# dotchen/LAV

Measured on AMD Instinct MI355X. Metric: frames/s full agent fwd (32k-pt LiDAR + 3 cams), higher is better.
Workload: dtype f32 (convolution contractions on the matrix cores with f32 accumulate at the error of an fp32 dot product, DESIGN 4.3: the layers on the split-operand kernel - BEV backbone, heads, crop stems, the brake net's mid-size layers - and ERFNet's persistent runs of pairs as two power-of-two-scaled fp16 pie

## Files before the change

### include/lav_amd.h

```cpp
#ifndef LAV_AMD_H
#define LAV_AMD_H

#include <stddef.h>
#include <stdint.h>

#ifdef __cplusplus
extern "C" {
#endif

#define LAV_ABI_VERSION 46

#define LAV_OK 0
#define LAV_EINVAL (-1)
#define LAV_EHIP (-2)
#define LAV_EWORKSPACE (-3)

int lav_abi_version(void);
const char *lav_last_error(void);
int lav_device_count(void);

int lav_profile_enable(int slots);
int lav_profile_reset(void);
int lav_profile_read(const char *kernel, double *total_ms, int *launches);

typedef struct lav_grid {
    float min_x, max_x, min_y, max_y;
    float ppm;
    int nx, ny;
} lav_grid;

typedef struct lav_pointnet {
    const float *w1, *b1, *w2, *b2;
    int num_input;
    int channels;
} lav_pointnet;

size_t lav_pillar_workspace_bytes(int batch, int max_points, const lav_grid *grid);
int lav_pillar_workspace_init(void *workspace, size_t workspace_bytes, void *stream);

int lav_pillar_scatter(const float *points, const int *h_num_points, int batch, int max_points, int D,
                       const lav_grid *grid, const lav_pointnet *net, float *canvas,
                       int *unique_coords, int *inverse, int *counts,
                       void *workspace, size_t workspace_bytes, void *stream);
int lav_pillar_amax_count(int batch, const lav_grid *grid);
int lav_pillar_scatter_amax(const float *points, const int *h_num_points, int batch, int max_points, int D,
                            const lav_grid *grid, const lav_pointnet *net, float *canvas,
                            int *unique_coords, int *inverse, int *counts, float *amax_parts,
                            void *workspace, size_t workspace_bytes, void *stream);

typedef struct lav_camera {
    float K[9];
    float l2w[16];
    float w2c[16];
} lav_camera;

int lav_paint(const float *lidar, int n, int lidar_dim, const float *sem, int ncam, int sem_c, int h, int w,
              const lav_camera *h_cams, float *fused, int *uvz, void *stream);

int lav_gru_cast(const float *embd, int B, int embd_dim, int H, int num_cmds, int T,
                 const float *w_ih, const float *w_hh, const float *b_ih, const float *b_hh,
                 const float *mlp_w, const float *mlp_b, float *out,
                 void *workspace, size_t workspace_bytes, void *stream);
size_t lav_gru_cast_workspace_bytes(int B, int embd_dim, int H, int num_cmds, int T);
// ... 141 lines not shown
int lav_bn_train_amax_count(int batch, int channels, long plane);
int lav_bn_train_forward_amax(const float *x, const float *residual, float *y, int batch, int channels, long plane, const float *gamma,
                              const float *beta, double eps, int relu_pre, int relu_post, float *save_mean, float *save_var,
                              float *save_rstd, float *amax_y, void *workspace, size_t workspace_bytes, void *stream);
int lav_bn_train_backward_amax(const float *x, const float *y, const float *dy, int batch, int channels, long plane, const float *gamma,
                               const float *save_mean, const float *save_rstd, int relu_pre, int relu_post, float *dx, float *dres,
                               float *dgamma, float *dbeta, float *amax_dx, void *workspace, size_t workspace_bytes, void *stream);

int lav_bn_train_forward_mask(const float *x, const float *residual, const float *chmask, float *y, int batch, int channels, long plane,
                              const float *gamma, const float *beta, double eps, int relu_post, float *save_mean, float *save_var,
                              float *save_rstd, float *amax_y, void *workspace, size_t workspace_bytes, void *stream);
int lav_bn_train_backward_mask(const float *x, const float *y, const float *dy, const float *chmask, int batch, int channels, long plane,
                               const float *gamma, const float *save_mean, const float *save_rstd, int relu_post, float *dx, float *dres,
                               float *dgamma, float *dbeta, float *amax_dx, void *workspace, size_t workspace_bytes, void *stream);

size_t lav_conv_wgrad_workspace_bytes(int batch, int cin, int cout, int h, int w, int ksize, int stride);
int lav_conv_wgrad(const float *x, const float *dy, int batch, int cin, int cout, int h, int w, int ksize, int stride, float *dw,
                   void *workspace, size_t workspace_bytes, void *stream);
int lav_conv_wgrad_amax(const float *x, const float *dy, int batch, int cin, int cout, int h, int w, int ksize, int stride, float *dw,
                        void *workspace, size_t workspace_bytes, const float *amax_x, int n_amax_x, const float *amax_dy, int n_amax_dy,
                        void *stream);

size_t lav_upconv_pointwise_packed_floats(int cin, int cout, int k);
int lav_upconv_pointwise_pack(int cin, int cout, int k, const float *h_weight, float *h_packed);
int lav_upconv_pointwise_parts(int batch, int cin, int cout, int ih, int iw, int k, int pad, int out_pad);
int lav_upconv_pointwise(int batch, int cin, int cout, int ih, int iw, int k, int pad, int out_pad, const float *x, const float *w_packed,
                         const float *scale, const float *shift, int relu_pre, int out_c_total, int out_c_offset, float *y,
                         float *amax_out, void *stream);

size_t lav_conv1d_pair_packed_weight_floats(int channels);
int lav_conv1d_pair_pack_weights(int channels, const float *h_weight, float *h_packed);
size_t lav_conv1d_pair_chain_workspace_bytes(int batch, int h);
size_t lav_conv1d_pair_chain_lds_bytes(int channels, int w, int d_b_max);
int lav_conv1d_pair_chain(int batch, int channels, int h, int w, int npairs, const int *d_a, const int *d_b, const int *residual,
                          const int *relu_post, const float *x, const float *const *wa_packed, const float *const *bias_a,
                          const float *const *wb_packed, const float *const *bias_b, const float *const *scale,
                          const float *const *shift, float *const *out, void *workspace, size_t workspace_bytes, void *stream);
int lav_conv1d_pair_chain_f16(int batch, int channels, int h, int w, int npairs, const int *d_a, const int *d_b, const int *residual,
                              const int *relu_post, const float *x, const float *const *wa_packed, const float *const *bias_a,
                              const float *const *wb_packed, const float *const *bias_b, const float *const *scale,
                              const float *const *shift, float *const *out, void *workspace, size_t workspace_bytes, void *stream);
int lav_conv1d_pair_chain_region(int row_offset, int clean_rows);
int lav_conv1d_pair_chain_status(const void *workspace, int *h_timeouts_launches2, void *stream);
size_t lav_conv1d_pair_lds_bytes(int channels, int w, int d_b);
size_t lav_conv3x3_run_f16_workspace_bytes(int channels, int h, int w, int nlayers);
size_t lav_conv3x3_run_f16_lds_bytes(int channels, int h, int w);
size_t lav_conv3x3_run_f16_weight_bytes(int channels);
int lav_conv3x3_run_f16_amax_count(int channels, int h, int w);
long lav_conv_f16_weights_offset(const lav_conv *c);
int lav_conv3x3_run_f16(int channels, int h, int w, int nlayers, const float *x, const void *const *w_f16, const float *const *scale,
                        const float *const *shift, float *out, const float *amax_in, int amax_in_count, float *amax_out, void *workspace,
                        size_t workspace_bytes, void *stream);
int lav_conv3x3_run_f16_status(const void *workspace, int *h_timeouts_launches2, void *stream);
size_t lav_conv3x3_tile_f16_lds_bytes(int channels, int h, int w, int nlayers);
int lav_conv3x3_tile_f16_amax_count(int channels, int h, int w, int nlayers);
int lav_conv3x3_tile_f16(int channels, int h, int w, int nlayers, const float *x, const void *const *w_f16, const float *const *scale,
                         const float *const *shift, float *out, const float *amax_in, int amax_in_count, float *amax_out, void *stream);
int lav_conv1d_pair(int batch, int channels, int h, int w, int d_a, int d_b, const float *x, const float *wa_packed,
                    const float *bias_a, const float *wb_packed, const float *bias_b, const float *scale, const float *shift,
                    const float *residual, int relu_post, float *y, void *stream);

int lav_pool_affine(const float *x, int batch, int channels, int h, int w, const float *scale, const float *shift, int relu,
                    float *y, int out_c_total, int out_c_offset, void *stream);

int lav_pair_train_supported(int channels, int width);
size_t lav_pair_train_workspace_bytes(int batch, int channels, int h);
int lav_pair_train_forward(const float *x, const float *wa, const float *ba, const float *wb, const float *bb, int batch, int channels,
                           int h, int w, int dil, float *t, float *z, void *stream);
int lav_pair_train_backward(const float *x, const float *t, const float *dz, const float *wa, const float *wb, int batch, int channels,
                            int h, int w, int dil, float *dt, float *dx, float *dwa, float *dba, float *dwb, float *dbb, void *workspace,
                            size_t workspace_bytes, void *stream);

size_t lav_seg_xent_workspace_bytes(void);
int lav_seg_xent_forward(const float *logits, const long long *labels, int batch, int classes, long plane, float *loss, float *dlogits,
                         void *workspace, size_t workspace_bytes, void *stream);

int lav_seg_xent_up_forward(const float *logits, const void *labels, int label_bytes, int batch, int classes, int h, int w, int scale,
                            float *loss, float *dlogits, void *workspace, size_t workspace_bytes, void *stream);

typedef struct lav_camera_f64 {
    double l2w[16];
    double w2c[16];
    double K[9];
} lav_camera_f64;

int lav_paint_frames(const float *lidar, const int *offsets, int frames, int total, int lidar_dim, const float *sem, int ncam,
                     int sem_c, int h, int w, const lav_camera_f64 *h_cams, float *painted, int *uvz, void *stream);

int lav_image_u8_to_f32(const unsigned char *img, int n, int h, int w, int c_src, int reverse, float *out, void *stream);

enum { LAV_AUG_BLUR = 0, LAV_AUG_NOISE = 1, LAV_AUG_DROPOUT = 2, LAV_AUG_MULTIPLY = 3, LAV_AUG_CONTRAST = 4, LAV_AUG_GRAYSCALE = 5,
       LAV_AUG_ELASTIC = 6, LAV_AUG_OPS = 7 };

typedef struct lav_augment_params {
    int order[7];
    int active;
    int per_channel;
    unsigned sample;
    unsigned tag;
    float blur_sigma;
    float blur_w[5];
    float noise_scale;
    float dropout_p;
    float multiply[3];
    float contrast[3];
    float gray_alpha;
    float elastic_alpha;
    float field_w[5];
} lav_augment_params;

int lav_augment_u8(const unsigned char *in, unsigned char *out, int n, int h, int w, const lav_augment_params *params,
                   unsigned long long seed, void *stream);

int lav_bev_stack_u8(const unsigned char *planes, const double *coef, const int *shift, unsigned char *out, int n, int h, int w,
                     int threshold, void *stream);
int lav_bev_stack_tile_paths(const double *coef, const int *shift, int h, int w, int *counts);
// ... 97 lines not shown
```

### lav_amd/_lib.py

```python
from __future__ import annotations

import ctypes as C
import os

HERE = os.path.dirname(os.path.abspath(__file__))
LIB_PATH = os.environ.get("LAV_AMD_LIB") or os.path.join(HERE, "liblav_amd.so")

ABI_VERSION = 46
MAX_CAM = 4
MAX_CAM_F64 = 8


class Grid(C.Structure):
    _fields_ = [("min_x", C.c_float), ("max_x", C.c_float), ("min_y", C.c_float), ("max_y", C.c_float),
                ("ppm", C.c_float), ("nx", C.c_int), ("ny", C.c_int)]


class PointNet(C.Structure):
    _fields_ = [("w1", C.c_void_p), ("b1", C.c_void_p), ("w2", C.c_void_p), ("b2", C.c_void_p),
                ("num_input", C.c_int), ("channels", C.c_int)]


class Camera(C.Structure):
    _fields_ = [("K", C.c_float * 9), ("l2w", C.c_float * 16), ("w2c", C.c_float * 16)]


class CameraF64(C.Structure):
    _fields_ = [("l2w", C.c_double * 16), ("w2c", C.c_double * 16), ("K", C.c_double * 9)]


class Conv(C.Structure):
    _fields_ = [(n, C.c_int) for n in (
        "batch", "in_c_total", "in_c_offset", "cin", "h", "w", "cout", "kh", "kw", "stride", "pad_h", "pad_w",
        "dil_h", "dil_w", "transposed", "out_pad", "out_c_total", "out_c_offset", "relu_pre", "relu_post", "sigmoid", "target_cus")] + [("pad_value", C.c_float), ("precision", C.c_int)]


CONV_F32, CONV_BF16X6, CONV_F16X3 = 1, 2, 3


_P, _I, _Z, _F = C.c_void_p, C.c_int, C.c_size_t, C.c_float
SIGNATURES = {
    "lav_abi_version": (_I, []),
    "lav_last_error": (C.c_char_p, []),
    "lav_device_count": (_I, []),
    "lav_profile_enable": (_I, [_I]),
    "lav_profile_reset": (_I, []),
    "lav_profile_read": (_I, [C.c_char_p, C.POINTER(C.c_double), C.POINTER(_I)]),
    "lav_pillar_workspace_bytes": (_Z, [_I, _I, C.POINTER(Grid)]),
    "lav_pillar_workspace_init": (_I, [_P, _Z, _P]),
    "lav_pillar_decorate_workspace_bytes": (_Z, [_I, _I, C.POINTER(Grid)]),
    "lav_pillar_scatter": (_I, [_P, C.POINTER(_I), _I, _I, _I, C.POINTER(Grid), C.POINTER(PointNet), _P, _P, _P, _P,
                                _P, _Z, _P]),
    "lav_pillar_amax_count": (_I, [_I, C.POINTER(Grid)]),
    "lav_pillar_scatter_amax": (_I, [_P, C.POINTER(_I), _I, _I, _I, C.POINTER(Grid), C.POINTER(PointNet), _P, _P, _P, _P, _P,
                                     _P, _Z, _P]),
    "lav_paint": (_I, [_P, _I, _I, _P, _I, _I, _I, _I, C.POINTER(Camera), _P, _P, _P]),
    "lav_paint_frames": (_I, [_P, _P, _I, _I, _I, _P, _I, _I, _I, _I, C.POINTER(CameraF64), _P, _P, _P]),
    "lav_image_u8_to_f32": (_I, [_P, _I, _I, _I, _I, _I, _P, _P]),
    "lav_gru_cast": (_I, [_P, _I, _I, _I, _I, _I, _P, _P, _P, _P, _P, _P, _P, _P, _Z, _P]),
    "lav_gru_cast_workspace_bytes": (_Z, [_I, _I, _I, _I, _I]),
    "lav_embed_cast": (_I, [_P, _I, _I, _I, _P, _I, _I, _I, _P, _P, _P, _P, _P, _P, _P, _P, _P, _P, _P, _P, _P]),
# ... 33 lines not shown
    "lav_upconv_pointwise_parts": (_I, [_I] * 8),
    "lav_upconv_pointwise": (_I, [_I] * 8 + [_P, _P, _P, _P, _I, _I, _I, _P, _P, _P]),
    "lav_conv1d_pair_chain_workspace_bytes": (_Z, [_I, _I]),
    "lav_conv1d_pair_chain_region": (_I, [_I, _I]),
    "lav_conv1d_pair_chain_lds_bytes": (_Z, [_I, _I, _I]),
    "lav_conv1d_pair_chain": (_I, [_I, _I, _I, _I, _I, C.POINTER(_I), C.POINTER(_I), C.POINTER(_I), C.POINTER(_I), _P] + [C.POINTER(_P)] * 7 + [_P, _Z, _P]),
    "lav_conv1d_pair_chain_f16": (_I, [_I, _I, _I, _I, _I, C.POINTER(_I), C.POINTER(_I), C.POINTER(_I), C.POINTER(_I), _P] + [C.POINTER(_P)] * 7 + [_P, _Z, _P]),
    "lav_conv1d_pair_chain_status": (_I, [_P, C.POINTER(_I), _P]),
    "lav_conv1d_pair_lds_bytes": (_Z, [_I, _I, _I]),
    "lav_conv3x3_run_f16_workspace_bytes": (_Z, [_I, _I, _I, _I]),
    "lav_conv3x3_run_f16_lds_bytes": (_Z, [_I, _I, _I]),
    "lav_conv3x3_run_f16_weight_bytes": (_Z, [_I]),
    "lav_conv3x3_run_f16_amax_count": (_I, [_I, _I, _I]),
    "lav_conv_f16_weights_offset": (C.c_long, [C.POINTER(Conv)]),
    "lav_conv3x3_run_f16": (_I, [_I, _I, _I, _I, _P, C.POINTER(_P), C.POINTER(_P), C.POINTER(_P), _P, _P, _I, _P, _P, _Z, _P]),
    "lav_conv3x3_run_f16_status": (_I, [_P, C.POINTER(_I), _P]),
    "lav_conv3x3_tile_f16_lds_bytes": (_Z, [_I, _I, _I, _I]),
    "lav_conv3x3_tile_f16_amax_count": (_I, [_I, _I, _I, _I]),
    "lav_conv3x3_tile_f16": (_I, [_I, _I, _I, _I, _P, C.POINTER(_P), C.POINTER(_P), C.POINTER(_P), _P, _P, _I, _P, _P]),
    "lav_conv1d_pair": (_I, [_I, _I, _I, _I, _I, _I, _P, _P, _P, _P, _P, _P, _P, _P, _I, _P, _P]),
    "lav_gru_seq_forward": (_I, [_P, _I, _P, _P, _P, _I, _I, _I, _P, _P, _P]),
    "lav_gru_seq_backward_workspace_bytes": (_Z, [_I, _I]),
    "lav_gru_seq_backward": (_I, [_P, _P, _P, _P, _P, _I, _I, _I, _P, _P, _P, _P, _Z, _P]),
    "lav_bn_train_workspace_bytes": (_Z, [_I]),
    "lav_bn_train_forward_mask": (_I, [_P, _P, _P, _P, _I, _I, C.c_long, _P, _P, C.c_double, _I, _P, _P, _P, _P, _P, _Z, _P]),
    "lav_bn_train_backward_mask": (_I, [_P, _P, _P, _P, _I, _I, C.c_long, _P, _P, _P, _I, _P, _P, _P, _P, _P, _P, _Z, _P]),
    "lav_pair_train_supported": (_I, [_I, _I]),
    "lav_pair_train_workspace_bytes": (_Z, [_I, _I, _I]),
    "lav_pair_train_forward": (_I, [_P, _P, _P, _P, _P, _I, _I, _I, _I, _I, _P, _P, _P]),
    "lav_pair_train_backward": (_I, [_P, _P, _P, _P, _P, _I, _I, _I, _I, _I, _P, _P, _P, _P, _P, _P, _P, _Z, _P]),
    "lav_seg_xent_workspace_bytes": (_Z, []),
    "lav_seg_xent_forward": (_I, [_P, _P, _I, _I, C.c_long, _P, _P, _P, _Z, _P]),
    "lav_seg_xent_up_forward": (_I, [_P, _P, _I, _I, _I, _I, _I, _I, _P, _P, _P, _Z, _P]),
    "lav_attn_train_workspace_bytes": (_Z, [_I, _I, _I, _I]),
    "lav_attn_train_forward": (_I, [_P, _I, _I, _I, _I, _P, _P, _P, _P, C.c_float, _P, _P, _P, _P, _P, _P]),
    "lav_attn_train_backward": (_I, [_P, _I, _I, _I, _I, _P, _P, _P, _P, C.c_float, _P, _P, _P, _P, _P, _P, _P, _P, _P, _Z, _P]),
    "lav_bn_train_forward": (_I, [_P, _P, _P, _I, _I, C.c_long, _P, _P, C.c_double, _I, _I, _P, _P, _P, _P, _Z, _P]),
    "lav_bn_train_backward": (_I, [_P, _P, _P, _I, _I, C.c_long, _P, _P, _P, _I, _I, _P, _P, _P, _P, _P, _Z, _P]),
    "lav_bn_train_amax_count": (_I, [_I, _I, C.c_long]),
    "lav_bn_train_forward_amax": (_I, [_P, _P, _P, _I, _I, C.c_long, _P, _P, C.c_double, _I, _I, _P, _P, _P, _P, _P, _Z, _P]),
    "lav_bn_train_backward_amax": (_I, [_P, _P, _P, _I, _I, C.c_long, _P, _P, _P, _I, _I, _P, _P, _P, _P, _P, _P, _Z, _P]),
    "lav_attn_pool": (_I, [_P, _I, _I, _I, _I, _P, _P, _P, _P, _P, _P]),
    "lav_linear_act": (_I, [_P, _I, _I, _P, _P, _I, _I, _P, _P]),
    "lav_maxpool3x3s2": (_I, [_P, _I, _I, _I, _I, _P, _P]),
    "lav_channel_affine": (_I, [_P, _I, _I, C.c_long, _P, _P, _P, _P]),
    "lav_nonfinite_count": (_I, [_I, C.POINTER(_P), C.POINTER(C.c_long), _P, _P]),
    "lav_copy_many": (_I, [_I, C.POINTER(_P), C.POINTER(_P), C.POINTER(_Z), _P]),
    "lav_stage_many": (_I, [_I, C.POINTER(_P), C.POINTER(_P), C.POINTER(_I), C.POINTER(C.c_long), C.POINTER(_I), _P]),
    "lav_det_decode": (_I, [_P, _I, _I, _I] + [C.c_double] * 10 + [_P, _P, _P]),
    "lav_det_decode_report": (_I, [_P, _I, _I, _I] + [C.c_double] * 10 + [_P, _P, _P, _P, _P, _P]),
    "lav_stage_many_block": (_I, [_I, C.POINTER(_P), C.POINTER(_P), C.POINTER(_I), C.POINTER(C.c_long), C.POINTER(_I), _P, _I, _P, _P]),
    "lav_batch_limit": (_I, [_P]),
    "lav_pool_affine": (_I, [_P, _I, _I, _I, _I, _P, _P, _I, _P, _I, _I, _P]),
    "lav_merge_ticks": (_I, [_P, _P, _I, _I, _P, _P]),
    "lav_stack_sweeps": (_I, [_P, _P, _P, _P, _P, _P, _I, _I, _I, _P, _P]),
    "lav_extract_peaks_workspace_bytes": (_Z, [_I, _I, _I]),
    "lav_extract_peaks": (_I, [_P, _I, _I, _I, _I, _I, _I, _P, _I, _P, _I, _P, _P, _Z, _P]),
    "lav_heads_at_peaks_packed_floats": (_Z, [_I, _I]),
    "lav_heads_at_peaks": (_I, [_P, _I, _I, _I, _P, _I, _I, _I, _P, _P, _P, _P, _P, _P, _P, _P, _P]),
    "lav_augment_u8": (_I, [_P, _P, _I, _I, _I, _P, C.c_ulonglong, _P]),
    "lav_bev_stack_u8": (_I, [_P, _P, _P, _P, _I, _I, _I, _I, _P]),
    "lav_bev_stack_tile_paths": (_I, [C.POINTER(C.c_double), C.POINTER(_I), _I, _I, C.POINTER(_I)]),
    "lav_debug_view": (_I, [_P, _I, _I, _P, _I, _I, _P, _I, _I, _P, _I, _P, _I, _P, _I, _P, _P, _P, C.c_double, C.c_double, _I, C.c_double, C.c_double, _I,
                            _I, _I, _P, _P, _P]),
    "lav_log_view": (_I, [_P, _I, _P, _I, _P, _P, _I, _I, _P, _P, _I, _P, _I, _I, _P, _P]),
    "lav_eval_acc_words": (_Z, [_I]),
    "lav_eval_frame": (_I, [_P, _P, _P, _I, _I, _F, _P, _I, _P, _P, _I, _I, _I, _P, _P, _I, _P, _P, _P, _I] + [C.c_double] * 6 + [_I, _P, _P]),
    "lav_eval_seg": (_I, [_P, _P, _I, _I, _I, _I, _I, _P, _P]),
    "lav_eval_scores": (_I, [_P, _P, _I, C.c_double, _I, _P, _P]),
    "lav_eval_plans_words": (_Z, [_I]),
    "lav_eval_plans": (_I, [_P, _P, _P, _P, _P, _P, _I, _I, _I, _P, _P, _P, _I, _P, _P]),
    "lav_eval_distill_words": (_Z, [_I]),
    "lav_eval_distill": (_I, [_P] * 8 + [_I, _I, _I] + [_P] * 5 + [_I, _P, _P]),
    "lav_eval_drive_words": (_Z, [_I]),
    "lav_eval_drive": (_I, [_P, _P, _P, _I, _I, _I, _I, _P, _P, _I, _P, _P, _I, _I] + [C.c_double] * 6 + [_I, _P, _P]),
    "lav_eval_det_words": (_Z, [_I]),
    "lav_eval_det": (_I, [_P, _I, _P, _P, _I, _I, _I, _P, _P, _I, _I] + [C.c_double] * 6 + [_P, _I, _P, _I, _P, _I, _I, _P, _P]),
    "lav_jpeg_scan_capacity": (C.c_longlong, [_I, _I, _I]),
    "lav_jpeg_workspace_bytes": (_Z, [_I, _I, _I, _I]),
    "lav_jpeg_encode": (_I, [_P, _I, _I, _I, _I, _P, _I, _P, C.c_longlong, _P, _P, _Z, _P]),
    "lav_optim_chunk": (_I, []),
    "lav_optim_workspace_bytes": (_Z, [C.c_longlong, C.c_longlong]),
    "lav_optim_grad_stats": (_I, [_P, _I, _I, _P, _I, _I, _P, C.c_double, _P, _Z, _P]),
    "lav_optim_adam_step": (_I, [_P, _I, _I, _P, _I, _I, _P, _P, C.c_double, _P, _Z, _P]),
}

_lib = None


def load() -> C.CDLL:
    global _lib
    if _lib is not None:
        return _lib
    if not os.path.exists(LIB_PATH):
        raise RuntimeError(
            f"{LIB_PATH} not found: build it with `python -m lav_amd.build` (hipcc, gfx950). "
            "lav_amd has no CPU or pure-torch fallback.")
    lib = C.CDLL(LIB_PATH)
    for name, (res, args) in SIGNATURES.items():
        fn = getattr(lib, name)
        fn.restype = res
        fn.argtypes = args
    got = lib.lav_abi_version()
    if got != ABI_VERSION:
        raise RuntimeError(f"liblav_amd ABI {got} != binding ABI {ABI_VERSION}: rebuild (python -m lav_amd.build --force)")
    _lib = lib
# ... 16 lines not shown
```

### lav_amd/build.py

```python
from __future__ import annotations

import os
import subprocess
import sys
import time

HERE = os.path.dirname(os.path.abspath(__file__))
REPO = os.path.dirname(HERE)
CSRC = os.path.join(HERE, "csrc")
LIB = os.path.join(HERE, "liblav_amd.so")
SOURCES = ["misc.hip", "pillar.hip", "paint.hip", "paint_frames.hip", "gru.hip", "gru_seq.hip", "conv.hip", "conv_f16.hip", "conv_pair.hip", "conv_run.hip", "conv_tile.hip", "deconv.hip", "crop.hip", "frame.hip", "heads_peaks.hip", "attn.hip", "bn_train.hip", "conv_wgrad.hip", "upconv.hip", "conv_pair_train.hip", "augment.hip", "bev_stack.hip", "debug_view.hip", "log_view.hip", "eval_metrics.hip", "eval_camera.hip", "eval_plans.hip", "eval_drive.hip", "eval_distill.hip", "eval_det.hip", "jpeg.hip", "optim.hip"]
EXTRA_FLAGS = {"pillar.hip": ["-ffp-contract=off"], "paint.hip": ["-ffp-contract=off"], "paint_frames.hip": ["-ffp-contract=off"], "crop.hip": ["-ffp-contract=off"],
               "frame.hip": ["-ffp-contract=off"], "augment.hip": ["-ffp-contract=off"], "bev_stack.hip": ["-ffp-contract=off"],
               "debug_view.hip": ["-ffp-contract=off", "-fhip-fp32-correctly-rounded-divide-sqrt"],
               "log_view.hip": ["-ffp-contract=off"],
               "eval_metrics.hip": ["-ffp-contract=off"],
               "eval_plans.hip": ["-ffp-contract=off"],
               "eval_drive.hip": ["-ffp-contract=off"],
               "eval_det.hip": ["-ffp-contract=off"],
               "eval_distill.hip": ["-ffp-contract=off"],
               "optim.hip": ["-ffp-contract=off", "-fhip-fp32-correctly-rounded-divide-sqrt"]}
FLAGS = ["--offload-arch=gfx950", "-O3", "-std=c++17", "-fPIC", "-Wall", "-Wno-unused-function", "-fno-slp-vectorize",
         "-I", os.path.join(REPO, "include"), "-I", CSRC]


def _hipcc() -> str:
    for c in (os.environ.get("HIPCC"), "/opt/rocm/bin/hipcc", "hipcc"):
        if c and (os.path.isabs(c) and os.path.exists(c) or not os.path.isabs(c)):
            return c
    raise RuntimeError("hipcc not found")


def needs_build() -> bool:
    if not os.path.exists(LIB):
        return True
    t = os.path.getmtime(LIB)
    deps = [os.path.join(CSRC, f) for f in os.listdir(CSRC)] + [os.path.join(REPO, "include", "lav_amd.h")]
    return any(os.path.getmtime(d) > t for d in deps)


def build(force: bool = False, verbose: bool = True) -> str:
    if not force and not needs_build():
        return LIB
    objs = []
    procs = []
    os.makedirs(os.path.join(HERE, "build"), exist_ok=True)
    t0 = time.time()
    for s in SOURCES:
        o = os.path.join(HERE, "build", s.replace(".hip", ".o"))
        objs.append(o)
        cmd = [_hipcc(), *FLAGS, *EXTRA_FLAGS.get(s, []), "-c", os.path.join(CSRC, s), "-o", o]
        procs.append((s, subprocess.Popen(cmd, stdout=subprocess.PIPE, stderr=subprocess.STDOUT, text=True)))
    for s, p in procs:
        out, _ = p.communicate()
        if p.returncode != 0:
            raise RuntimeError(f"hipcc failed on {s}:\n{out}")
        if verbose and out.strip():
            print(out)
    link = [_hipcc(), "--offload-arch=gfx950", "-shared", "-fPIC", *objs, "-o", LIB]
    r = subprocess.run(link, stdout=subprocess.PIPE, stderr=subprocess.STDOUT, text=True)
    if r.returncode != 0:
        raise RuntimeError("link failed:\n" + r.stdout)
    if verbose:
        print(f"built {LIB} in {time.time() - t0:.1f}s")
# ... 6 lines not shown
```

### lav_amd/erfnet.py

```python
from __future__ import annotations

import os

import torch
import torch.nn as nn
import torch.nn.functional as F

from . import ops
from .engine import Engine
from .ops import Conv1dPair, Conv1dPairChain, ConvLayer, GroupedDeconv, infer_precision

_USE_PAIRS = os.environ.get("LAV_ERFNET_PAIRS", "1") != "0"


def _affine(bn, sl):
    s, t = ops.bn_fold(bn.running_mean, bn.running_var, bn.weight, bn.bias, bn.eps)
    return s[sl].float()[None, :, None, None].contiguous(), t[sl].float()[None, :, None, None].contiguous()


class DownsamplerBlock(nn.Module):
    def __init__(self, cin, cout):
        super().__init__()
        self.conv = nn.Conv2d(cin, cout - cin, 3, stride=2, padding=1, bias=True)
        self.pool = nn.MaxPool2d(2, stride=2)
        self.bn = nn.BatchNorm2d(cout, eps=1e-3)

    def forward(self, x):
        return F.relu(self.bn(torch.cat([self.conv(x), self.pool(x)], 1)))

    def engine(self, device, input_affine=None):
        from . import ops
        nconv = self.conv.out_channels
        cout = self.bn.num_features
        w, b, pad = self.conv.weight.detach(), self.conv.bias.detach(), 0.0
        s_in, t_in = (1.0, 0.0) if input_affine is None else input_affine
        if input_affine is not None:
            if not s_in > 0:
                raise RuntimeError("input_affine needs a positive scale")
            b = (b.double() + t_in * w.double().sum(dim=(1, 2, 3))).float()
            w = (w.double() * s_in).float()
            pad = -t_in / s_in
        sl = slice(0, nconv)
        bn = tuple(t[sl] for t in (self.bn.running_mean, self.bn.running_var, self.bn.weight, self.bn.bias))
        conv = ConvLayer(w, stride=2, padding=(1, 1), bias=b, bn=bn, bn_eps=self.bn.eps, relu_post=True, out_c_total=cout,
                         pad_value=pad, device=device)
        ps, pt = _affine(self.bn, slice(nconv, cout))
        ps, pt = ps.reshape(-1).double(), pt.reshape(-1).double()
        ps, pt = (ps * s_in).float().to(device), (pt + ps * t_in).float().to(device)

        def run(x):
            out = conv(x)
            return ops.pool_affine(x, ps, pt, out, nconv, relu=True)
        return run


class non_bottleneck_1d(nn.Module):
    def __init__(self, ch, dropprob, dilated):
        super().__init__()
        d = dilated
        self.conv3x1_1 = nn.Conv2d(ch, ch, (3, 1), padding=(1, 0))
        self.conv1x3_1 = nn.Conv2d(ch, ch, (1, 3), padding=(0, 1))
        self.bn1 = nn.BatchNorm2d(ch, eps=1e-3)
        self.conv3x1_2 = nn.Conv2d(ch, ch, (3, 1), padding=(d, 0), dilation=(d, 1))
        self.conv1x3_2 = nn.Conv2d(ch, ch, (1, 3), padding=(0, d), dilation=(1, d))
        self.bn2 = nn.BatchNorm2d(ch, eps=1e-3)
        self.dropout = nn.Dropout2d(dropprob)

    def forward(self, x):
        if self.training and x.is_cuda:
            from .train.hipnn import nb1d_train
            return nb1d_train(self, x)
        return self.forward_torch(x)

    def forward_torch(self, x):
        y = F.relu(self.bn1(self.conv1x3_1(F.relu(self.conv3x1_1(x)))))
        y = self.bn2(self.conv1x3_2(F.relu(self.conv3x1_2(y))))
        if self.dropout.p != 0:
            y = self.dropout(y)
        return F.relu(y + x)

    def engine(self, device):
        a = ConvLayer.from_module(self.conv3x1_1, relu_post=True, device=device)
        b = ConvLayer.from_module(self.conv1x3_1, self.bn1, relu_post=True, device=device)
        c = ConvLayer.from_module(self.conv3x1_2, relu_post=True, device=device)
        d = ConvLayer.from_module(self.conv1x3_2, self.bn2, relu_post=True, device=device)
        p1 = Conv1dPair(self.conv3x1_1, self.conv1x3_1, self.bn1, device=device)
        p2 = Conv1dPair(self.conv3x1_2, self.conv1x3_2, self.bn2, device=device)

        def run(x):
            if _USE_PAIRS and p1.supported(x) and p2.supported(x):
                return p2(p1(x), residual=x)
            return d(c(b(a(x))), residual=x)
        run.pairs = (p1, p2)
        return run


def _chain_blocks(stages):
    out, run = [], []

    def flush():
        if not run:
            return
        blocks = list(run)
        run.clear()
        if len(blocks) == 1 or not _USE_PAIRS:
            out.extend(blocks)
# ... 27 lines not shown
    def __init__(self, cin, cout):
        super().__init__()
        self.conv = nn.ConvTranspose2d(cin, cout, 3, stride=2, padding=1, output_padding=1, bias=True)
        self.bn = nn.BatchNorm2d(cout, eps=1e-3)

    def forward(self, x):
        return F.relu(self.bn(self.conv(x)))

    def engine(self, device):
        return ConvLayer.from_module(self.conv, self.bn, relu_post=True, device=device)


class Encoder(nn.Module):
    def __init__(self, num_classes):
        super().__init__()
        self.initial_block = DownsamplerBlock(3, 16)
        blocks = [DownsamplerBlock(16, 64)] + [non_bottleneck_1d(64, 0.03, 1) for _ in range(5)] + [DownsamplerBlock(64, 128)]
        blocks += [non_bottleneck_1d(128, 0.3, d) for _ in range(2) for d in (2, 4, 8, 16)]
        self.layers = nn.ModuleList(blocks)
        self.output_conv = nn.Conv2d(128, num_classes, 1)

    def forward(self, x, predict=False):
        x = self.initial_block(x)
        for layer in self.layers:
            x = layer(x)
        return self.output_conv(x) if predict else x


class Decoder(nn.Module):
    def __init__(self, num_classes):
        super().__init__()
        self.layers = nn.ModuleList([UpsamplerBlock(128, 64), non_bottleneck_1d(64, 0, 1), non_bottleneck_1d(64, 0, 1),
                                     UpsamplerBlock(64, 16), non_bottleneck_1d(16, 0, 1), non_bottleneck_1d(16, 0, 1)])
        self.output_conv = nn.ConvTranspose2d(16, num_classes, 2, stride=2)

    def forward(self, x):
        for layer in self.layers:
            x = layer(x)
        return self.output_conv(x)


class ERFNet(Engine):
    def __init__(self, num_classes):
        super().__init__()
        self.encoder = Encoder(num_classes)
        self.decoder = Decoder(num_classes)

    _mark_stale = Engine._drop

    def _engine(self, device, input_affine=None, softmax=False):
        def build():
            stages = [self.encoder.initial_block.engine(device, input_affine)]
            stages += [m.engine(device) for m in self.encoder.layers]
            stages += [m.engine(device) for m in self.decoder.layers]
            stages = _chain_blocks(stages)
            stages.append(GroupedDeconv([self.decoder.output_conv], softmax=softmax, device=device))
            return stages
        return self._engine_for(device, (input_affine, softmax, infer_precision()), build)

    def chains(self, precision):
        return [s.chain for key, stages in (self.__dict__.get("_eng") or {}).items() if isinstance(key, tuple) and key[2] == precision
                for s in stages if getattr(s, "chain", None) is not None]

    def forward(self, x, input_affine=None, softmax=False):
        if self.training:
            if input_affine is not None:
                x = x * input_affine[0] + input_affine[1]
            y = self.decoder(self.encoder(x))
            return torch.softmax(y, dim=1) if softmax else y
        if not x.is_cuda:
            raise RuntimeError("ERFNet: eval-mode forward needs a tensor in HBM - lav_amd has no CPU path "
                               "(CPU evaluation for tests and baselines: oracle/camera.py)")
        shared = os.environ.get("LAV_CHAIN_SHARED_CLEAN", "1") != "0"
        cap, off, first = ops.pair_chain_capacity(x.device), 0, True
        for stage in self._engine(x.device, input_affine, softmax):
            chain = getattr(stage, "chain", None)
            rows = x.shape[0] * x.shape[2]
            if shared and chain is not None and chain.supported(x) and off + rows <= cap:
                with ops.pair_chain_region(off, cap if first else 0):
                    x = stage(x)
                off, first = off + rows, False
            else:
                if chain is not None:
                    shared = False
                x = stage(x)
        return x
```

### lav_amd/ops.py

```python
from __future__ import annotations

import ctypes as C
import functools
import os as _os
import threading as _threading
from typing import Optional, Sequence

import numpy as np
import torch

from . import _lib
from ._lib import Camera, Conv, Grid, PointNet, check

_workspaces: dict = {}


def _stream() -> int:
    return torch.cuda.current_stream().cuda_stream


def _ptr(t: Optional[torch.Tensor]) -> Optional[int]:
    return None if t is None else t.data_ptr()


# ... 1573 lines not shown
        nb = bsrc.numel() * bsrc.element_size()
        if (stage and not bsrc.is_cuda and bsrc.is_contiguous() and bdst.is_cuda and bdst.is_contiguous() and nb % 4 == 0 and 0 < nb <= 256
                and nb == bdst.numel() * bdst.element_size() and bdst.data_ptr() % 4 == 0):
            blk = (bsrc.data_ptr(), nb, bdst.data_ptr())
        else:
            bdst.copy_(bsrc, non_blocking=True)
    for i in range(0, len(stage), 8):
        part = stage[i:i + 8]
        n = len(part)
        dims, strides = [], []
        for dst, src in part:
            pad = 4 - src.dim()
            dims += [1] * pad + list(src.shape)
            strides += [0] * pad + list(src.stride())
        b = blk if i == 0 else (None, 0, None)
        check(lib.lav_stage_many_block(n, (C.c_void_p * n)(*[s_.data_ptr() for _, s_ in part]), (C.c_void_p * n)(*[d.data_ptr() for d, _ in part]),
                                       (C.c_int * (4 * n))(*dims), (C.c_long * (4 * n))(*strides),
                                       (C.c_int * n)(*[int(s_.dtype == torch.uint8) for _, s_ in part]), b[0], b[1], b[2], _stream()), "lav_stage_many")


def linear_act(x: torch.Tensor, weight: torch.Tensor, bias, sigmoid: bool = False) -> torch.Tensor:
    x = _f32c(x, "x")
    B, K = x.shape
    O = weight.shape[0]
    out = torch.empty((B, O), dtype=torch.float32, device=x.device)
    check(_lib.load().lav_linear_act(_ptr(x), B, K, _ptr(_f32c(weight, "weight")), _ptr(None if bias is None else _f32c(bias, "bias")), O,
                                     int(bool(sigmoid)), _ptr(out), _stream()), "lav_linear_act")
    return out


def attn_pool(x: torch.Tensor, u: torch.Tensor, dots_bias: torch.Tensor, w_v: torch.Tensor, b_v: torch.Tensor, heads: int,
              out: Optional[torch.Tensor] = None) -> torch.Tensor:
    x = _f32c(x, "x")
    B, Cc, H, W = x.shape
    if out is None:
        out = torch.empty((B, Cc), dtype=torch.float32, device=x.device)
    elif tuple(out.shape) != (B, Cc) or out.dtype != torch.float32 or not out.is_cuda or (B > 1 and out.stride(0) != Cc) or out.stride(1) != 1:
        raise RuntimeError("attn_pool: out must be a (B, C) float32 buffer in HBM with rows C apart")
    check(_lib.load().lav_attn_pool(_ptr(x), B, Cc, H * W, int(heads), _ptr(_f32c(u, "u")), _ptr(_f32c(dots_bias, "dots_bias")),
                                    _ptr(_f32c(w_v, "w_v")), _ptr(_f32c(b_v, "b_v")), _ptr(out), _stream()), "lav_attn_pool")
    return out


def pool_affine(x: torch.Tensor, scale: torch.Tensor, shift: torch.Tensor, out: torch.Tensor, out_c_offset: int, relu: bool = True):
    x = _f32c(x, "x")
    B, Cc, H, W = x.shape
    if out.shape[0] != B or out.shape[2:] != (H // 2, W // 2) or not out.is_contiguous():
        raise RuntimeError("pool_affine: output buffer does not match")
    check(_lib.load().lav_pool_affine(_ptr(x), B, Cc, H, W, _ptr(_f32c(scale, "scale")), _ptr(_f32c(shift, "shift")), int(relu),
                                      _ptr(out), out.shape[1], int(out_c_offset), _stream()), "lav_pool_affine")
    return out


def crop_rotate(features: torch.Tensor, locs: torch.Tensor, oris: torch.Tensor, pixels_per_meter: float, crop: int,
                offset_x: float, offset_y: float) -> torch.Tensor:
    lib = _lib.load()
    features, locs, oris, out = _crop_args(features, locs, oris, crop)
    fb, Cc, H, W = features.shape
    n = locs.shape[0]
    if fb not in (1, n):
        raise RuntimeError("features batch must be 1 (shared map) or N")
    check(lib.lav_crop_rotate(_ptr(features), fb, Cc, H, W, _ptr(locs), _ptr(oris), n, float(pixels_per_meter), int(crop),
                              float(offset_x), float(offset_y), _ptr(out), _stream()), "lav_crop_rotate")
    return out


def merge_ticks(tick: torch.Tensor, prev: torch.Tensor, out: torch.Tensor | None = None) -> torch.Tensor:
    lib = _lib.load()
    tick, prev = _f32c(tick, "tick"), _f32c(prev, "prev")
    if tick.shape != prev.shape or tick.dim() != 2 or tick.shape[1] != 4:
        raise RuntimeError(f"merge_ticks: tick {tuple(tick.shape)} / prev {tuple(prev.shape)} must both be (P, 4)")
    P = tick.shape[0]
    if out is None:
        out = torch.empty((2 * P, 4), dtype=torch.float32, device=tick.device)
    check(lib.lav_merge_ticks(_ptr(tick), _ptr(prev), P, 4, _ptr(out), _stream()), "lav_merge_ticks")
    return out


def stack_sweeps(fused: torch.Tensor, ring: torch.Tensor, slot: torch.Tensor, sweeps: torch.Tensor, R: torch.Tensor,
                 t: torch.Tensor, out: torch.Tensor | None = None) -> torch.Tensor:
    lib = _lib.load()
    fused, ring, R, t = _f32c(fused, "fused"), _f32c(ring, "ring"), _f32c(R, "R"), _f32c(t.reshape(-1, 3), "t")
    S, rows, dim = sweeps.numel(), fused.shape[0], fused.shape[1]
    if ring.shape[1:] != fused.shape or slot.dtype != torch.long or sweeps.dtype != torch.long or R.shape != (S, 3, 3):
        raise RuntimeError("stack_sweeps: inconsistent arguments")
    if out is None:
        out = torch.empty((S * rows, dim + S), dtype=torch.float32, device=fused.device)
    check(lib.lav_stack_sweeps(_ptr(fused), _ptr(ring), _ptr(slot), _ptr(sweeps), _ptr(R), _ptr(t), S, rows, dim, _ptr(out),
                               _stream()), "lav_stack_sweeps")
    return out


def extract_peaks(heat: torch.Tensor, size: Optional[torch.Tensor] = None, ori: Optional[torch.Tensor] = None, ks: int = 7,
                  max_det: int = 15, apply_sigmoid: bool = False) -> torch.Tensor:
    lib = _lib.load()
    heat = _f32c(heat, "heat")
    size, ori = (None if size is None else _f32c(size, "size")), (None if ori is None else _f32c(ori, "ori"))
    ncls, H, W = heat.shape
    if any(m is not None and m.shape[1:] != (H, W) for m in (size, ori)):
        raise RuntimeError("extract_peaks: size / ori maps must match the heat map")
    cs, co = (0 if size is None else size.shape[0]), (0 if ori is None else ori.shape[0])
    out = torch.empty((ncls, max_det, 3 + cs + co), dtype=torch.float32, device=heat.device)
    nbytes = lib.lav_extract_peaks_workspace_bytes(ncls, H, W)
    ws = _workspace("peaks", nbytes, heat.device)
    check(lib.lav_extract_peaks(_ptr(heat), ncls, H, W, ks, max_det, int(apply_sigmoid), _ptr(size), cs, _ptr(ori), co, _ptr(out),
                                _ptr(ws), ws.numel(), _stream()), "lav_extract_peaks")
# ... 67 lines not shown
```

Baseline: 553.8.

## Fuse ERFNet initial block and first downsampler into one entry kernel

Adds a single HIP kernel that computes ERFNet's initial downsampler (3->16, conv plus maxpool, BN, ReLU) and the first 16->64 downsampler (conv on MFMA f32 plus maxpool, BN, ReLU) per 8x8 output tile. The half-resolution intermediate stays in LDS with a halo, so it is never written to or read back from HBM, and several launches collapse into one. The cost is recomputing halo rows, a large LDS footprint that may limit occupancy, and the loss of the separate-stage paths whenever the fused path is chosen.

```diff
diff --git a/include/lav_amd.h b/include/lav_amd.h
--- a/include/lav_amd.h
+++ b/include/lav_amd.h
@@ -8,7 +8,7 @@
 extern "C" {
 #endif
 
-#define LAV_ABI_VERSION 46
+#define LAV_ABI_VERSION 47
 
 #define LAV_OK 0
 #define LAV_EINVAL (-1)
@@ -256,6 +256,7 @@
                         const float *const *shift, float *out, const float *amax_in, int amax_in_count, float *amax_out, void *workspace,
                         size_t workspace_bytes, void *stream);
 int lav_conv3x3_run_f16_status(const void *workspace, int *h_timeouts_launches2, void *stream);
+
 size_t lav_conv3x3_tile_f16_lds_bytes(int channels, int h, int w, int nlayers);
 int lav_conv3x3_tile_f16_amax_count(int channels, int h, int w, int nlayers);
 int lav_conv3x3_tile_f16(int channels, int h, int w, int nlayers, const float *x, const void *const *w_f16, const float *const *scale,
@@ -266,6 +267,10 @@
 
 int lav_pool_affine(const float *x, int batch, int channels, int h, int w, const float *scale, const float *shift, int relu,
                     float *y, int out_c_total, int out_c_offset, void *stream);
+
+int lav_erfnet_entry(const float *x, int batch, int h, int w, const float *w1, const float *b1, float pad_value, const float *scale1,
+                     const float *shift1, const float *w2, const float *b2, const float *scale2, const float *shift2, float *y,
+                     void *stream);
 
 int lav_pair_train_supported(int channels, int width);
 size_t lav_pair_train_workspace_bytes(int batch, int channels, int h);
diff --git a/lav_amd/_lib.py b/lav_amd/_lib.py
--- a/lav_amd/_lib.py
+++ b/lav_amd/_lib.py
@@ -6,7 +6,7 @@
 HERE = os.path.dirname(os.path.abspath(__file__))
 LIB_PATH = os.environ.get("LAV_AMD_LIB") or os.path.join(HERE, "liblav_amd.so")
 
-ABI_VERSION = 46
+ABI_VERSION = 47
 MAX_CAM = 4
 MAX_CAM_F64 = 8
 
@@ -146,6 +146,7 @@
     "lav_stage_many_block": (_I, [_I, C.POINTER(_P), C.POINTER(_P), C.POINTER(_I), C.POINTER(C.c_long), C.POINTER(_I), _P, _I, _P, _P]),
     "lav_batch_limit": (_I, [_P]),
     "lav_pool_affine": (_I, [_P, _I, _I, _I, _I, _P, _P, _I, _P, _I, _I, _P]),
+    "lav_erfnet_entry": (_I, [_P, _I, _I, _I, _P, _P, _F, _P, _P, _P, _P, _P, _P, _P, _P]),
     "lav_merge_ticks": (_I, [_P, _P, _I, _I, _P, _P]),
     "lav_stack_sweeps": (_I, [_P, _P, _P, _P, _P, _P, _I, _I, _I, _P, _P]),
     "lav_extract_peaks_workspace_bytes": (_Z, [_I, _I, _I]),
diff --git a/lav_amd/build.py b/lav_amd/build.py
--- a/lav_amd/build.py
+++ b/lav_amd/build.py
@@ -9,7 +9,7 @@
 REPO = os.path.dirname(HERE)
 CSRC = os.path.join(HERE, "csrc")
 LIB = os.path.join(HERE, "liblav_amd.so")
-SOURCES = ["misc.hip", "pillar.hip", "paint.hip", "paint_frames.hip", "gru.hip", "gru_seq.hip", "conv.hip", "conv_f16.hip", "conv_pair.hip", "conv_run.hip", "conv_tile.hip", "deconv.hip", "crop.hip", "frame.hip", "heads_peaks.hip", "attn.hip", "bn_train.hip", "conv_wgrad.hip", "upconv.hip", "conv_pair_train.hip", "augment.hip", "bev_stack.hip", "debug_view.hip", "log_view.hip", "eval_metrics.hip", "eval_camera.hip", "eval_plans.hip", "eval_drive.hip", "eval_distill.hip", "eval_det.hip", "jpeg.hip", "optim.hip"]
+SOURCES = ["misc.hip", "pillar.hip", "paint.hip", "paint_frames.hip", "gru.hip", "gru_seq.hip", "conv.hip", "conv_f16.hip", "conv_pair.hip", "conv_run.hip", "conv_tile.hip", "deconv.hip", "crop.hip", "frame.hip", "heads_peaks.hip", "attn.hip", "bn_train.hip", "conv_wgrad.hip", "upconv.hip", "conv_pair_train.hip", "augment.hip", "bev_stack.hip", "debug_view.hip", "log_view.hip", "eval_metrics.hip", "eval_camera.hip", "eval_plans.hip", "eval_drive.hip", "eval_distill.hip", "eval_det.hip", "jpeg.hip", "optim.hip", "erfnet_edge.hip"]
 EXTRA_FLAGS = {"pillar.hip": ["-ffp-contract=off"], "paint.hip": ["-ffp-contract=off"], "paint_frames.hip": ["-ffp-contract=off"], "crop.hip": ["-ffp-contract=off"],
                "frame.hip": ["-ffp-contract=off"], "augment.hip": ["-ffp-contract=off"], "bev_stack.hip": ["-ffp-contract=off"],
                "debug_view.hip": ["-ffp-contract=off", "-fhip-fp32-correctly-rounded-divide-sqrt"],
diff --git a/lav_amd/csrc/erfnet_edge.hip b/lav_amd/csrc/erfnet_edge.hip
--- /dev/null
+++ b/lav_amd/csrc/erfnet_edge.hip
@@ -0,0 +1,197 @@
+#include <cstdint>
+
+#include "common.hpp"
+
+namespace {
+using namespace lav;
+typedef float f32x4 __attribute__((ext_vector_type(4)));
+
+constexpr int EN_T = 8;
+constexpr int EN_RN = 2 * EN_T + 1;
+constexpr int EN_PN = 4 * EN_T + 3;
+constexpr int EN_IS = 37;
+constexpr int EN_RS = 24;
+constexpr int EN_CS = EN_RN * EN_RS + 1;
+constexpr int EN_WS = 49;
+constexpr int EN_C1 = 16, EN_C1C = 13, EN_C2 = 64, EN_C2C = 48, EN_K1 = 27, EN_K2 = 144;
+constexpr int EN_IN = (3 * EN_PN * EN_IS + 3) / 4 * 4, EN_B1 = EN_C1 * EN_CS, EN_W2 = EN_K2 * EN_WS, EN_W1 = EN_K1 * EN_C1;
+constexpr int EN_EP = 3 * EN_C1 + EN_C2C + 2 * EN_C2;
+constexpr size_t EN_LDS = (size_t)(EN_IN + EN_B1 + EN_W2 + EN_W1 + EN_EP) * sizeof(float);
+
+struct EntryArgs {
+    const float *__restrict__ x, *__restrict__ w1, *__restrict__ b1, *__restrict__ s1, *__restrict__ t1;
+    const float *__restrict__ w2, *__restrict__ b2, *__restrict__ s2, *__restrict__ t2;
+    float *__restrict__ y;
+    int H, W;
+    float pad;
+};
+
+__global__ __launch_bounds__(256) void k_erfnet_entry(EntryArgs a) {
+    extern __shared__ __attribute__((aligned(16))) float en_smem[];
+    float *s_in = en_smem;
+    float *s_b1 = s_in + EN_IN;
+    float *s_w2 = s_b1 + EN_B1;
+    float *s_w1 = s_w2 + EN_W2;
+    float *s_ep = s_w1 + EN_W1;
+    const int tid = threadIdx.x, lane = tid & 63, wave = __builtin_amdgcn_readfirstlane(tid >> 6);
+    const int n = blockIdx.z, oy0 = blockIdx.y * EN_T, ox0 = blockIdx.x * EN_T;
+    const int H = a.H, W = a.W, H1 = H >> 1, W1 = W >> 1, OH = H >> 2, OW = W >> 2;
+
+    {
+        const int iy0 = 4 * oy0 - 3, ix0 = 4 * ox0 - 3;
+        const float *xn = a.x + (long)n * 3 * H * W;
+        constexpr int NPT = 3 * EN_PN * EN_PN, NIT = (NPT + 255) / 256;
+        float v[NIT];
+#pragma unroll
+        for (int i = 0; i < NIT; ++i) {
+            const int e = min(tid + 256 * i, NPT - 1);
+            const int px = e % EN_PN, r = e / EN_PN, py = r % EN_PN, ci = r / EN_PN;
+            const int iy = iy0 + py, ix = ix0 + px;
+            const bool ok = iy >= 0 && iy < H && ix >= 0 && ix < W;
+            const float t = xn[((long)ci * H + min(max(iy, 0), H - 1)) * W + min(max(ix, 0), W - 1)];
+            v[i] = ok ? t : a.pad;
+        }
+        constexpr int NW4 = EN_C2C * EN_K2 / 4, NWI = (NW4 + 255) / 256;
+        float4 wv[NWI];
+#pragma unroll
+        for (int i = 0; i < NWI; ++i) wv[i] = reinterpret_cast<const float4 *>(a.w2)[min(tid + 256 * i, NW4 - 1)];
+#pragma unroll
+        for (int i = 0; i < NIT; ++i) {
+            const int e = tid + 256 * i;
+            if (e < NPT) s_in[(e / EN_PN) * EN_IS + e % EN_PN] = v[i];
+        }
+#pragma unroll
+        for (int i = 0; i < NWI; ++i) {
+            const int q = tid + 256 * i;
+            if (q < NW4) {
+                const float w4[4] = {wv[i].x, wv[i].y, wv[i].z, wv[i].w};
+#pragma unroll
+                for (int j = 0; j < 4; ++j) {
+                    const int e = 4 * q + j, tap = e % 9, r = e / 9, ci = r % 16, co = r / 16;
+                    s_w2[(tap * 16 + ci) * EN_WS + co] = w4[j];
+                }
+            }
+        }
+        for (int d = tid; d < EN_W1; d += 256) {
+            const int co = d % EN_C1, k = d / EN_C1;
+            s_w1[d] = co < EN_C1C ? a.w1[co * EN_K1 + k] : 0.f;
+        }
+        if (tid < EN_C1) {
+            s_ep[tid] = tid < EN_C1C ? a.b1[tid] : 0.f;
+            s_ep[EN_C1 + tid] = a.s1[tid];
+            s_ep[2 * EN_C1 + tid] = a.t1[tid];
+        }
+        if (tid < EN_C2C) s_ep[3 * EN_C1 + tid] = a.b2[tid];
+        if (tid < EN_C2) {
+            s_ep[3 * EN_C1 + EN_C2C + tid] = a.s2[tid];
+            s_ep[3 * EN_C1 + EN_C2C + EN_C2 + tid] = a.t2[tid];
+        }
+    }
+    __syncthreads();
+
+    {
+        const int c0 = 4 * wave;
+        const float4 b4 = *reinterpret_cast<const float4 *>(s_ep + c0), sc4 = *reinterpret_cast<const float4 *>(s_ep + EN_C1 + c0),
+                     sh4 = *reinterpret_cast<const float4 *>(s_ep + 2 * EN_C1 + c0);
+        const float bb[4] = {b4.x, b4.y, b4.z, b4.w}, ss[4] = {sc4.x, sc4.y, sc4.z, sc4.w}, hh[4] = {sh4.x, sh4.y, sh4.z, sh4.w};
+        for (int p = lane; p < EN_RN * EN_RN; p += 64) {
+            const int ry = p / EN_RN, rx = p - ry * EN_RN;
+            const int y1 = 2 * oy0 - 1 + ry, x1 = 2 * ox0 - 1 + rx;
+            const bool inside = y1 >= 0 && y1 < H1 && x1 >= 0 && x1 < W1;
+            const float *in0 = s_in + (2 * ry) * EN_IS + 2 * rx;
+            float acc[4] = {0.f, 0.f, 0.f, 0.f};
+#pragma unroll
+            for (int ci = 0; ci < 3; ++ci)
+#pragma unroll
+                for (int ky = 0; ky < 3; ++ky)
+#pragma unroll
+                    for (int kx = 0; kx < 3; ++kx) {
+                        const float xv = in0[(ci * EN_PN + ky) * EN_IS + kx];
+                        const float4 w4 = *reinterpret_cast<const float4 *>(s_w1 + (ci * 9 + ky * 3 + kx) * EN_C1 + c0);
+                        acc[0] = fmaf(xv, w4.x, acc[0]);
+                        acc[1] = fmaf(xv, w4.y, acc[1]);
+                        acc[2] = fmaf(xv, w4.z, acc[2]);
+                        acc[3] = fmaf(xv, w4.w, acc[3]);
+                    }
+            float v[4];
+#pragma unroll
+            for (int j = 0; j < 4; ++j) v[j] = acc[j] + bb[j];
+            if (wave == 3) {
+#pragma unroll
+                for (int c = 0; c < 3; ++c) {
+                    const float *q = in0 + (c * EN_PN + 1) * EN_IS + 1;
+                    v[c + 1] = fmaxf(fmaxf(q[0], q[1]), fmaxf(q[EN_IS], q[EN_IS + 1]));
+                }
+            }
+#pragma unroll
+            for (int j = 0; j < 4; ++j) {
+                float t = fmaf(v[j], ss[j], hh[j]);
+                t = t > 0.f ? t : 0.f;
+                s_b1[(c0 + j) * EN_CS + ry * EN_RS + rx] = inside ? t : 0.f;
+            }
+        }
+    }
+    __syncthreads();
+
+    const long plane = (long)OH * OW;
+    float *yn = a.y + (long)n * EN_C2 * plane;
+    {
+        const int pr = lane & 15, kq = lane >> 4;
+        const int py = 2 * wave + (pr >> 3), px = pr & 7;
+        const float *xb = s_b1 + kq * EN_CS + (2 * py) * EN_RS + 2 * px;
+        const float *wb = s_w2 + kq * EN_WS + pr;
+        f32x4 acc[3] = {f32x4{0.f, 0.f, 0.f, 0.f}, f32x4{0.f, 0.f, 0.f, 0.f}, f32x4{0.f, 0.f, 0.f, 0.f}};
+#pragma unroll
+        for (int tap = 0; tap < 9; ++tap)
+#pragma unroll
+            for (int kc = 0; kc < 4; ++kc) {
+                const float xv = xb[4 * kc * EN_CS + (tap / 3) * EN_RS + tap % 3];
+                const float *wr = wb + (tap * 16 + 4 * kc) * EN_WS;
+#pragma unroll
+                for (int nt = 0; nt < 3; ++nt) acc[nt] = __builtin_amdgcn_mfma_f32_16x16x4f32(wr[16 * nt], xv, acc[nt], 0, 0, 0);
+            }
+        const int oy = oy0 + py, ox = ox0 + px;
+        if (oy < OH && ox < OW) {
+            const float *e_b = s_ep + 3 * EN_C1, *e_s = e_b + EN_C2C, *e_t = e_s + EN_C2;
+#pragma unroll
+            for (int nt = 0; nt < 3; ++nt)
+#pragma unroll
+                for (int j = 0; j < 4; ++j) {
+                    const int co = 16 * nt + 4 * kq + j;
+                    float v = acc[nt][j] + e_b[co];
+                    v = fmaf(v, e_s[co], e_t[co]);
+                    yn[co * plane + (long)oy * OW + ox] = v > 0.f ? v : 0.f;
+                }
+        }
+    }
+    {
+        const float *e_s = s_ep + 3 * EN_C1 + EN_C2C + EN_C2C, *e_t = e_s + EN_C2;
+#pragma unroll
+        for (int i = 0; i < 4; ++i) {
+            const int it = tid + 256 * i, px = it & 7, py = (it >> 3) & 7, c = it >> 6;
+            const float *q = s_b1 + c * EN_CS + (2 * py + 1) * EN_RS + 2 * px + 1;
+            float v = fmaxf(fmaxf(q[0], q[1]), fmaxf(q[EN_RS], q[EN_RS + 1]));
+            v = fmaf(v, e_s[c], e_t[c]);
+            const int oy = oy0 + py, ox = ox0 + px;
+            if (oy < OH && ox < OW) yn[(EN_C2C + c) * plane + (long)oy * OW + ox] = v > 0.f ? v : 0.f;
+        }
+    }
+}
+}
+
+extern "C" int lav_erfnet_entry(const float *x, int batch, int h, int w, const float *w1, const float *b1, float pad_value, const float *scale1,
+                                const float *shift1, const float *w2, const float *b2, const float *scale2, const float *shift2, float *y,
+                                void *stream) {
+    LAV_REQUIRE(batch >= 1 && batch <= 65535 && h >= 4 && w >= 4 && h % 4 == 0 && w % 4 == 0, "lav_erfnet_entry: h, w multiples of 4 and 1 <= batch <= 65535 expected");
+    LAV_REQUIRE((long)batch * 64 * (h / 4) * (w / 4) < (1L << 31) && (long)batch * 3 * h * w < (1L << 31), "lav_erfnet_entry: tensor too large");
+    LAV_REQUIRE(x && w1 && b1 && scale1 && shift1 && w2 && b2 && scale2 && shift2 && y, "lav_erfnet_entry: bad argument");
+    LAV_REQUIRE(reinterpret_cast<uintptr_t>(w2) % 16 == 0, "lav_erfnet_entry: w2 must be 16-byte aligned");
+    hipStream_t st = static_cast<hipStream_t>(stream);
+    EntryArgs a{x, w1, b1, scale1, shift1, w2, b2, scale2, shift2, y, h, w, pad_value};
+    const dim3 grid((unsigned)((w / 4 + EN_T - 1) / EN_T), (unsigned)((h / 4 + EN_T - 1) / EN_T), (unsigned)batch);
+    LAV_REQUIRE(grid.y <= 65535, "lav_erfnet_entry: image too tall");
+    const int tok = timer_begin("erfnet_entry", st);
+    const int rc = launch_lds<k_erfnet_entry>(grid, dim3(256), EN_LDS, st, (int)EN_LDS, a);
+    timer_end(tok, st);
+    return rc;
+}
diff --git a/lav_amd/erfnet.py b/lav_amd/erfnet.py
--- a/lav_amd/erfnet.py
+++ b/lav_amd/erfnet.py
@@ -10,6 +10,7 @@
 from .engine import Engine
 from .ops import Conv1dPair, Conv1dPairChain, ConvLayer, GroupedDeconv, infer_precision
 
+ERFNET_ENTRY_DEFAULT = "1"
 _USE_PAIRS = os.environ.get("LAV_ERFNET_PAIRS", "1") != "0"
 
 
@@ -28,10 +29,8 @@
     def forward(self, x):
         return F.relu(self.bn(torch.cat([self.conv(x), self.pool(x)], 1)))
 
-    def engine(self, device, input_affine=None):
-        from . import ops
-        nconv = self.conv.out_channels
-        cout = self.bn.num_features
+    def _folded(self, input_affine=None):
+        nconv, cout = self.conv.out_channels, self.bn.num_features
         w, b, pad = self.conv.weight.detach(), self.conv.bias.detach(), 0.0
         s_in, t_in = (1.0, 0.0) if input_affine is None else input_affine
         if input_affine is not None:
@@ -40,18 +39,44 @@
             b = (b.double() + t_in * w.double().sum(dim=(1, 2, 3))).float()
             w = (w.double() * s_in).float()
             pad = -t_in / s_in
+        ps, pt = _affine(self.bn, slice(nconv, cout))
+        ps, pt = ps.reshape(-1).double(), pt.reshape(-1).double()
+        return w, b, pad, (ps * s_in).float(), (pt + ps * t_in).float()
+
+    def engine(self, device, input_affine=None):
+        nconv = self.conv.out_channels
+        cout = self.bn.num_features
+        w, b, pad, ps, pt = self._folded(input_affine)
         sl = slice(0, nconv)
         bn = tuple(t[sl] for t in (self.bn.running_mean, self.bn.running_var, self.bn.weight, self.bn.bias))
         conv = ConvLayer(w, stride=2, padding=(1, 1), bias=b, bn=bn, bn_eps=self.bn.eps, relu_post=True, out_c_total=cout,
                          pad_value=pad, device=device)
-        ps, pt = _affine(self.bn, slice(nconv, cout))
-        ps, pt = ps.reshape(-1).double(), pt.reshape(-1).double()
-        ps, pt = (ps * s_in).float().to(device), (pt + ps * t_in).float().to(device)
+        ps, pt = ps.to(device), pt.to(device)
 
         def run(x):
             out = conv(x)
             return ops.pool_affine(x, ps, pt, out, nconv, relu=True)
         return run
+
+
+def _entry_stage(b1, b2, device, input_affine, first, second):
+    def vectors(m, ps, pt):
+        nconv = m.conv.out_channels
+        s, t = ops.bn_fold(*[v.detach().cpu()[:nconv] for v in (m.bn.running_mean, m.bn.running_var, m.bn.weight, m.bn.bias)], m.bn.eps)
+        return torch.cat([s.float(), ps.cpu()]).to(device), torch.cat([t.float(), pt.cpu()]).to(device)
+    w1, bias1, pad, ps1, pt1 = b1._folded(input_affine)
+    w2, bias2, _, ps2, pt2 = b2._folded()
+    s1, t1 = vectors(b1, ps1, pt1)
+    s2, t2 = vectors(b2, ps2, pt2)
+    w1, bias1, w2, bias2 = (v.to(device, torch.float32).contiguous() for v in (w1, bias1, w2, bias2))
+
+    def run(x):
+        if ops.erfnet_entry_takes(x):
+            return ops.erfnet_entry(x, w1, bias1, pad, s1, t1, w2, bias2, s2, t2)
+        return second(first(x))
+    run.fused_entry = True
+    run.args = (w1, bias1, pad, s1, t1, w2, bias2, s2, t2)
+    return run
 
 
 class non_bottleneck_1d(nn.Module):
@@ -185,6 +210,10 @@
         def build():
             stages = [self.encoder.initial_block.engine(device, input_affine)]
             stages += [m.engine(device) for m in self.encoder.layers]
+            ib, l0 = self.encoder.initial_block, self.encoder.layers[0]
+            if (os.environ.get("LAV_ERFNET_ENTRY", ERFNET_ENTRY_DEFAULT) != "0" and isinstance(l0, DownsamplerBlock)
+                    and (ib.conv.in_channels, ib.bn.num_features, l0.bn.num_features) == (3, 16, 64)):
+                stages[:2] = [_entry_stage(ib, l0, device, input_affine, stages[0], stages[1])]
             stages += [m.engine(device) for m in self.decoder.layers]
             stages = _chain_blocks(stages)
             stages.append(GroupedDeconv([self.decoder.output_conv], softmax=softmax, device=device))
diff --git a/lav_amd/ops.py b/lav_amd/ops.py
--- a/lav_amd/ops.py
+++ b/lav_amd/ops.py
@@ -1649,6 +1649,31 @@
     return out
 
 
+def erfnet_entry_takes(x: torch.Tensor) -> bool:
+    return (x.dim() == 4 and x.is_cuda and x.dtype == torch.float32 and x.is_contiguous() and x.shape[1] == 3 and 1 <= x.shape[0] <= 65535
+            and x.shape[2] >= 4 and x.shape[3] >= 4 and x.shape[2] % 4 == 0 and x.shape[3] % 4 == 0 and x.shape[2] <= 8 * 4 * 65535)
+
+
+def erfnet_entry(x: torch.Tensor, w1, b1, pad_value: float, scale1, shift1, w2, b2, scale2, shift2, out: Optional[torch.Tensor] = None):
+    if not erfnet_entry_takes(x):
+        raise RuntimeError(f"erfnet_entry: input {tuple(x.shape)} is not served (contiguous float32 (B,3,H,W) with H, W multiples of 4)")
+    B, _, H, W = x.shape
+    if out is None:
+        out = torch.empty((B, 64, H // 4, W // 4), dtype=torch.float32, device=x.device)
+    elif tuple(out.shape) != (B, 64, H // 4, W // 4) or out.dtype != torch.float32 or not out.is_contiguous() or out.device != x.device:
+        raise RuntimeError("erfnet_entry: output buffer does not match")
+    vec = [("w1", w1, 13 * 27), ("b1", b1, 13), ("scale1", scale1, 16), ("shift1", shift1, 16), ("w2", w2, 48 * 144), ("b2", b2, 48),
+           ("scale2", scale2, 64), ("shift2", shift2, 64)]
+    ptrs = {}
+    for name, t, n in vec:
+        if t.numel() != n or t.device != x.device:
+            raise RuntimeError(f"erfnet_entry: {name} must hold {n} floats on {x.device}")
+        ptrs[name] = _ptr(_f32c(t, name))
+    check(_lib.load().lav_erfnet_entry(_ptr(x), B, H, W, ptrs["w1"], ptrs["b1"], float(pad_value), ptrs["scale1"], ptrs["shift1"], ptrs["w2"],
+                                       ptrs["b2"], ptrs["scale2"], ptrs["shift2"], _ptr(out), _stream()), "lav_erfnet_entry")
+    return out
+
+
 def crop_rotate(features: torch.Tensor, locs: torch.Tensor, oris: torch.Tensor, pixels_per_meter: float, crop: int,
                 offset_x: float, offset_y: float) -> torch.Tensor:
     lib = _lib.load()
```

New measurement: 569.4, median of 6. 1.03x the previous value.
